# harukaki/brl

Hardware: AMD Instinct MI355X
Metric: env-steps/sec at num_envs=8192, 32-step rollout, 1/2/4/8 MI355X (higher is better)
Workload: dtype u8

## Files before the change

brl_amd/_capi.py:

```python
from __future__ import annotations

import ctypes as C
import os

_PKG = os.path.dirname(os.path.abspath(__file__))
LIB_PATH = os.path.join(_PKG, "lib", "libbrl_hip.so")

STATE_WORDS = 16
OBS_SIZE = 480
NUM_ACTIONS = 38

_vp = C.c_void_p


class Fields(C.Structure):
    _names = ["current_player", "terminated", "rewards", "step_count", "turn", "dealer", "vul_ns", "vul_ew",
              "shuffled_players", "last_bid", "last_bidder", "call_x", "call_xx", "pass_num",
              "first_denomination_ns", "first_denomination_ew", "hand", "tricks", "lut_idx", "board_ctr", "illegal"]
    _fields_ = [(n, _vp) for n in _names]


class TransitionPtrs(C.Structure):
    _names = ["done", "action", "value", "reward", "log_prob", "obs", "legal_action_mask"]
    _fields_ = [(n, _vp) for n in _names]
# ... 95 lines not shown
        "brl_ppo_stats": [i32, _vp, i64, _vp, f32, f32, _vp, _vp],
        "brl_ppo_heads_loss_split": [i32, _vp, i64, _vp, _vp, i64, _vp, _vp, _vp, _vp, _vp, _vp, i64, f32, f32, f32, i32, i32, i32, _vp, _vp, _vp, _vp, _vp, i32, _vp],
        "brl_ppo_heads_bwd": [i32, _vp, _vp, i64, _vp, i64, i64, i32, i32, _vp, _vp, _vp, _vp, _vp, _vp, i64, _vp, _vp, _vp, _vp],
        "brl_ppo_stats_rows": [i32, _vp, _vp, i64, i64, f32, f32, f32, _vp, _vp],
        "brl_mb_gather_bind": [i32, C.POINTER(TransitionPtrs), _vp, _vp, _vp, _vp, i64, _vp, _vp, _vp, _vp, _vp, _vp, _vp, i64, _vp, _vp],
        "brl_adam_clip_fin_gather": [i32, _vp, _vp, _vp, _vp, i64, _vp, f32, _vp, f32, f32, f32, f32, _vp, i64, _vp, _vp, _vp, i64,
                                     i32, _vp, _vp, _vp, _vp, _vp],
        "brl_mb_gather_dev": [i32, _vp, i64, _vp],
        "brl_ppo_stats_gram": [i32, _vp, i64, i64, _vp, i64, f32, f32, f32, _vp, _vp, _vp, _vp],
        "brl_ppo_illegal_grad": [i32, _vp, _vp, _vp, f32, i64, _vp, _vp],
        "brl_act_bwd_colsum": [i32, _vp, _vp, i64, i64, i64, i32, _vp, _vp],
        "brl_act_bwd_colsum_heads_dw": [i32, _vp, _vp, i64, i64, i64, i32, _vp, _vp, _vp, i64, i64, i64, i32, _vp, _vp, _vp, _vp, i64,
                                        _vp, _vp, _vp, _vp],
        "brl_bias_finalize_ex": [i32, i32, _vp, _vp, _vp, _vp, _vp],
        "brl_bias_finalize_rows": [i32, i32, _vp, _vp, _vp, _vp, i32, _vp, _vp],
        "brl_fair_forward": [i32, C.POINTER(FairNet), _vp, i64, i32, _vp, _vp, _vp],
        "brl_mlp_gemm_group": [i32, i32, i32, _vp, _vp, _vp, _vp, _vp, _vp, _vp, _vp, _vp, _vp],
        "brl_fair_chain": [i32, C.POINTER(FairNet), _vp, _vp, _vp, _vp, _vp, _vp, _vp, i64, f32, f32, f32, i32, i32, i32, i32,
                           C.POINTER(FairWork), _vp],
        "brl_mlp_gemm": [i32, i32, i32, _vp, i64, _vp, i64, _vp, i64, i64, i64, i64, i32, _vp, _vp, i64, _vp, _vp, _vp],
        "brl_mlp_gemm_x3_workspace": [i64, i64, i64, _vp],
        "brl_mlp_gemm_x3_group": [i32, i32, i32, _vp, _vp, _vp, _vp, _vp, _vp, _vp, _vp, _vp, _vp],
        "brl_split_planes": [i32, _vp, i64, _vp, i64, _vp],
        "brl_linear_x3p": [i32, _vp, i32, i64, i64, _vp, i64, i64, _vp, i32, _vp, i64, _vp, i64, i64, i64, i64, i64, _vp],
        "brl_mlp_gemm_x3": [i32, i32, i32, _vp, i64, _vp, i64, _vp, i64, i64, i64, i64, i32, _vp, _vp, i64, _vp, _vp, i64, _vp],
        "brl_mlp_forward_rows": [i32, C.POINTER(MlpRef), _vp, _vp, i64, _vp, i64, _vp, i64, _vp],
        "brl_adam_shard_norm": [i32, _vp, C.POINTER(ShardGeom), i32, i32, f32, _vp, _vp, _vp, _vp],
        "brl_adam_shard_apply": [i32, _vp, _vp, _vp, _vp, C.POINTER(ShardGeom), i32, i32, _vp, _vp, f32, _vp, f32, f32, f32, f32, f32, _vp,
                                 _vp, i64, _vp],
        "brl_mlp_gemm_dh_heads_dw": [i32, _vp, i64, _vp, i64, _vp, i64, i64, i64, i64, i32, _vp, i64, _vp, _vp, _vp, i64, i64, i64, i32,
                                     _vp, _vp, _vp, _vp, i64, _vp, _vp, _vp, _vp],
    }
    sigs.update(sl_signatures())
    for name, args in sigs.items():
        fn = getattr(L, name)
        fn.argtypes = args
        fn.restype = i32
    _lib = L
    return L


EXPORTS = ["brl_last_error", "brl_version", "brl_create", "brl_set_lut", "brl_destroy", "brl_set_rng",
           "brl_init_random", "brl_init_from_deals", "brl_step", "brl_observe", "brl_get_fields",
           "brl_rollout_random", "brl_policy_step", "brl_policy_step_at", "brl_obs_cast", "brl_obs_cast_rows", "brl_live_index", "brl_linear_act", "brl_linear_act_heads", "brl_gae", "brl_imp_reward", "brl_duplicate_step",
           "brl_eval_step", "brl_eval_reduce", "brl_ppo_loss", "brl_ppo_stats", "brl_policy_step_ex",
           "brl_eval_step_team", "brl_rollout_random_gae", "brl_ppo_heads_loss_split", "brl_adam_shard_norm", "brl_adam_shard_apply", "brl_ppo_heads_bwd", "brl_ppo_stats_gram",
           "brl_act_bwd_colsum", "brl_act_bwd_colsum_heads_dw", "brl_bias_finalize_ex", "brl_ppo_stats_rows", "brl_mb_gather_bind", "brl_mb_gather_dev", "brl_ppo_illegal_grad", "brl_adam_clip_fin_gather", "brl_mlp_gemm", "brl_mlp_gemm_dh_heads_dw", "brl_mlp_forward_rows",
           "brl_bias_finalize_rows", "brl_fair_chain", "brl_mlp_gemm_group", "brl_fair_forward", "brl_mlp_gemm_x3", "brl_mlp_gemm_x3_workspace", "brl_mlp_gemm_x3_group", "brl_split_planes", "brl_linear_x3p"]


def sl_signatures() -> dict:
    i64, i32, u64, f32 = C.c_int64, C.c_int, C.c_uint64, C.c_float
    return {
        "brl_sl_sample": [i32, _vp, _vp, i64, u64, i64, _vp, _vp, _vp],
        "brl_sl_replay": [i32, _vp, _vp, _vp, i64, _vp, _vp, i64, _vp, _vp, _vp, _vp],
        "brl_sl_loss": [i32, _vp, i64, _vp, _vp, i64, f32, _vp, _vp, _vp, i64, _vp],
    }


def check(rc: int) -> None:
    if rc != 0:
        raise BrlError(f"libbrl_hip error {rc}: {lib().brl_last_error().decode()}")


def ptr(t):
    if t is None:
        return None
    assert t.is_contiguous(), "brl_amd passes raw pointers: tensors must be contiguous"
    return t.data_ptr()
```

brl_amd/csrc/brl_mlp_gemm_x3.hip:

```cpp
#include <hip/hip_runtime.h>
#include <stdint.h>

#include "abi_common.hpp"
#include "mlp_gemm_x3.hpp"
#include "mlp_linear_x3p.hpp"

static int64_t x3_tiles(int64_t m, int64_t n) { return ((m + 127) / 128) * ((n + 127) / 128); }

static int64_t x3_workspace_bytes(int64_t m, int64_t n, int64_t k) {
  const int sk = mgs::pick_splitk(m, n, k);
  if (sk == 1) return 0;
  const int64_t tiles = x3_tiles(m, n);
  return ((tiles * 4 + 255) / 256) * 256 + tiles * sk * (int64_t)mgs::SLAB_FLOATS * 4;
}

extern "C" int brl_mlp_gemm_x3_workspace(int64_t m, int64_t n, int64_t k, int64_t *bytes) {
  NEED(bytes && m > 0 && n > 0 && k > 0, "bytes / m / n / k");
  *bytes = x3_workspace_bytes(m, n, k);
  return BRL_OK;
}

extern "C" int brl_mlp_gemm_x3(int device, int layout, int epilogue, const float *a, int64_t lda, const float *b, int64_t ldb, float *c,
                               int64_t ldc, int64_t m, int64_t n, int64_t k, int act, const float *bias, const float *gate, int64_t ldg,
                               float *colsum, void *workspace, int64_t workspace_bytes, void *stream) {
  NEED(a && b && c && m > 0 && n > 0 && k > 0, "a / b / c / m / n / k");
  NEED(layout >= BRL_GEMM_NT && layout <= BRL_GEMM_TN, "layout (BRL_GEMM_NT / _NN / _TN)");
  NEED(m < (1 << 24) && n < (1 << 24) && k < (1 << 24), "m / n / k below 2^24");
  NEED(n % 4 == 0 && ldc % 4 == 0 && lda % 4 == 0 && ldb % 4 == 0 && ldc >= n, "n and the leading dimensions multiples of 4 (16-byte pieces)");
  const bool akc = layout != BRL_GEMM_TN, bkc = layout == BRL_GEMM_NT;
  NEED(k % 32 == 0, "k a multiple of 32 (whole 32-deep chunks; other k: brl_mlp_gemm)");
  NEED(akc ? lda >= k : lda >= ((m + 3) & ~(int64_t)3), "lda (where m is contiguous in a: at least m rounded up to 4 — whole 16-byte pieces are read)");
  NEED(bkc ? ldb >= k : ldb >= n, "ldb");
  NEED((akc ? m * lda : k * lda) < (1ll << 29) && (bkc ? n * ldb : k * ldb) < (1ll << 29), "operands below 2 GB");
  NEED(act == 0 || act == 1, "act (0 ReLU, 1 tanh)");
  NEED((epilogue == BRL_GEMM_EPI_NONE) || (epilogue == BRL_GEMM_EPI_BIAS_ACT && layout == BRL_GEMM_NT && bias) ||
           (epilogue == BRL_GEMM_EPI_GATE_COLSUM && layout == BRL_GEMM_NN && gate && ldg >= n && ldg % 4 == 0),
// ... 44 lines not shown
    NEED(m[i] < (1 << 24) && n[i] < (1 << 24) && k[i] < (1 << 24), "m / n / k below 2^24");
    NEED(n[i] % 4 == 0 && ldc[i] % 4 == 0 && lda[i] % 4 == 0 && ldb[i] % 4 == 0 && ldc[i] >= n[i], "n and the leading dimensions multiples of 4");
    NEED(k[i] % 32 == 0, "k a multiple of 32 (whole 32-deep chunks; other k: brl_mlp_gemm_group)");
    NEED(akc ? lda[i] >= k[i] : lda[i] >= ((m[i] + 3) & ~(int64_t)3), "lda (where m is contiguous in a: at least m rounded up to 4)");
    NEED(bkc ? ldb[i] >= k[i] : ldb[i] >= n[i], "ldb");
    NEED((akc ? m[i] * lda[i] : k[i] * lda[i]) < (1ll << 29) && (bkc ? n[i] * ldb[i] : k[i] * ldb[i]) < (1ll << 29), "operands below 2 GB");
    NEED((((uintptr_t)a[i] | (uintptr_t)b[i] | (uintptr_t)c[i]) & 15) == 0, "16-byte alignment");
    mgs::Args &X = GA.x[i];
    mg::Args &G = X.g;
    G.A = a[i]; G.lda = lda[i]; G.B = b[i]; G.ldb = ldb[i]; G.C = c[i]; G.ldc = ldc[i];
    G.M = (int)m[i]; G.N = (int)n[i]; G.K = (int)k[i];
    X.splitk = 1;
    GA.first[i + 1] = GA.first[i] + (int)x3_tiles(m[i], n[i]);
  }
  HIP_TRY(hipSetDevice(device));
  hipStream_t s = (hipStream_t)stream;
  const unsigned blocks = (unsigned)GA.first[count];
  if (layout == BRL_GEMM_NT) hipLaunchKernelGGL((mgs::k_gemm_x3s_group<true, true>), dim3(blocks), dim3(mgs::THREADS), 0, s, GA);
  else if (layout == BRL_GEMM_NN) hipLaunchKernelGGL((mgs::k_gemm_x3s_group<true, false>), dim3(blocks), dim3(mgs::THREADS), 0, s, GA);
  else hipLaunchKernelGGL((mgs::k_gemm_x3s_group<false, false>), dim3(blocks), dim3(mgs::THREADS), 0, s, GA);
  HIP_TRY(hipGetLastError());
  return BRL_OK;
}

extern "C" int brl_split_planes(int device, const float *x, int64_t n, uint16_t *planes, int64_t plane_stride, void *stream) {
  NEED(x && planes && n > 0 && n % 4 == 0 && plane_stride >= n && plane_stride % 4 == 0, "x / planes / n (a multiple of 4) / plane_stride");
  NEED((((uintptr_t)x) & 15) == 0 && (((uintptr_t)planes) & 7) == 0, "alignment (x 16 bytes, planes 8)");
  HIP_TRY(hipSetDevice(device));
  hipLaunchKernelGGL(lx3::k_split_planes, dim3((unsigned)((n / 4 + 255) / 256)), dim3(256), 0, (hipStream_t)stream, x, planes, plane_stride, n / 4);
  HIP_TRY(hipGetLastError());
  return BRL_OK;
}

extern "C" int brl_linear_x3p(int device, const uint16_t *x_planes, int npx, int64_t ldx, int64_t sx, const uint16_t *w_planes, int64_t ldw,
                              int64_t sw, const float *bias, int relu, float *y, int64_t ldy, uint16_t *y_planes, int64_t ldyp, int64_t syp,
                              int64_t m, int64_t n, int64_t k, void *stream) {
  NEED(x_planes && w_planes && bias && (y || y_planes) && m > 0 && n > 0 && k > 0, "x_planes / w_planes / bias / an output / m / n / k");
  NEED(npx == 1 || npx == 3, "npx (3 planes, or 1: x exact in bf16)");
  NEED(n % 128 == 0 && k % 32 == 0, "n a multiple of 128, k a multiple of 32");
  NEED(m < (1 << 24) && n < (1 << 24) && k < (1 << 24), "m / n / k below 2^24");
  NEED(ldx >= k && ldx % 8 == 0 && ldw >= k && ldw % 8 == 0, "ldx / ldw (at least k, multiples of 8: 16-byte pieces)");
  NEED(m * ldx < (1ll << 31) && n * ldw < (1ll << 31), "planes below 4 GB each");
  NEED(!y || (ldy >= n && ldy % 4 == 0), "ldy");
  NEED(!y_planes || (ldyp >= n && ldyp % 8 == 0 && syp % 8 == 0), "ldyp / syp (multiples of 8)");
  NEED(sx % 8 == 0 && sw % 8 == 0, "plane strides multiples of 8");
  NEED((((uintptr_t)x_planes | (uintptr_t)w_planes | (uintptr_t)bias | (uintptr_t)y | (uintptr_t)y_planes) & 15) == 0, "16-byte alignment");
  HIP_TRY(hipSetDevice(device));
  lx3::Args G{};
  G.x = x_planes; G.ldx = ldx; G.sx = sx; G.w = w_planes; G.ldw = ldw; G.sw = sw; G.bias = bias;
  G.y = y; G.ldy = ldy; G.yp = y_planes; G.ldyp = ldyp; G.syp = syp;
  G.M = (int)m; G.N = (int)n; G.K = (int)k; G.relu = relu ? 1 : 0;
  hipStream_t s = (hipStream_t)stream;
  const unsigned blocks = (unsigned)(((m + 127) / 128) * (n / 128));
  if (npx == 3) hipLaunchKernelGGL(lx3::k_linear_x3p<3>, dim3(blocks), dim3(lx3::THREADS), 0, s, G);
  else hipLaunchKernelGGL(lx3::k_linear_x3p<1>, dim3(blocks), dim3(lx3::THREADS), 0, s, G);
  HIP_TRY(hipGetLastError());
  return BRL_OK;
}
```

brl_amd/csrc/mlp_linear_x3p.hpp:

```cpp
#pragma once

#include "mlp_gemm.hpp"

namespace lx3 {

using mg::f32x4;
typedef __bf16 bf16x8 __attribute__((ext_vector_type(8)));
typedef float f32x16 __attribute__((ext_vector_type(16)));
typedef unsigned u32x4 __attribute__((ext_vector_type(4)));
typedef unsigned u32x2 __attribute__((ext_vector_type(2)));

constexpr int BK = 32, STAGES = 3, THREADS = 512;
constexpr int PLANE = 128 * 64;
constexpr int STAGE_BYTES = 6 * PLANE;
constexpr int LDS_BYTES = STAGES * STAGE_BYTES;
constexpr int C_ROW_BYTES = 128 * 2 + 16;
static_assert(3 * 128 * C_ROW_BYTES <= LDS_BYTES, "the output planes reuse the stages");

struct Args {
  const uint16_t *x;
  int64_t ldx, sx;
  const uint16_t *w;
  int64_t ldw, sw;
  const float *bias;
  float *y;
  int64_t ldy;
  uint16_t *yp;
  int64_t ldyp, syp;
  int M, N, K;
  int relu;
#ifdef LX3_TIMING
  unsigned long long *dbg;
#endif
};
#ifdef LX3_TIMING
#define LX3_STAMP(k) do { if (threadIdx.x == 0 && G.dbg) { G.dbg[(size_t)blockIdx.x * 4 + 2 * (k)] = __builtin_amdgcn_s_memtime(); \
                                                          G.dbg[(size_t)blockIdx.x * 4 + 2 * (k) + 1] = __builtin_amdgcn_s_memrealtime(); } } while (0)
#else
#define LX3_STAMP(k) do { } while (0)
#endif

template <bool V>
struct BoolTag { static constexpr bool value = V; };

#ifndef LX3_STORE
#define LX3_STORE 0
#endif
#ifndef LX3_EXP
#define LX3_EXP 0
#endif

__device__ __forceinline__ void glds16(const void *g, void *lds_wave_base) {
  __builtin_amdgcn_global_load_lds((const __attribute__((address_space(1))) void *)g, (__attribute__((address_space(3))) void *)lds_wave_base, 16,
                                   0, 0);
}

__device__ __forceinline__ void split3(const float x, unsigned &hi, unsigned &mid, unsigned &lo) {
  const unsigned u = __float_as_uint(x);
  const float r = x - __uint_as_float(u & 0xffff0000u);
  const unsigned ur = __float_as_uint(r);
  const float l = r - __uint_as_float(ur & 0xffff0000u);
  hi = u >> 16;
  mid = ur >> 16;
  lo = __float_as_uint(l) >> 16;
}

template <int NPX>
__global__ __launch_bounds__(THREADS) void k_linear_x3p(Args G) {
  static_assert(NPX == 1 || NPX == 3, "x: one plane (exact in bf16) or three");
  constexpr int NI = NPX + 3;
  constexpr int NP = NPX == 3 ? 6 : 3;
  constexpr int NMF = 4 * NP;
  constexpr int NFR = 2 * NPX + 3;
  __shared__ __attribute__((aligned(16))) unsigned char lds[LDS_BYTES];
  const int tid = (int)threadIdx.x, lane = tid & 63, w = __builtin_amdgcn_readfirstlane(tid >> 6);
  const int tiles_m = (G.M + 127) / 128, tiles_n = G.N / 128, nblk = (int)gridDim.x, bid = (int)blockIdx.x;
  const int L = (nblk % 8 == 0) ? (bid % 8) * (nblk / 8) + bid / 8 : bid;
  int tm, tn;
  if (tiles_m % 2 == 0 && tiles_n % 4 == 0) {
    const int blk = L >> 3, i = L & 7;
    tm = 2 * (blk / (tiles_n / 4)) + (i >> 2);
    tn = 4 * (blk % (tiles_n / 4)) + (i & 3);
  } else {
    tm = L / tiles_n;
    tn = L - tm * tiles_n;
  }
  const int m0 = tm * 128, n0 = tn * 128;
  const int nchunks = G.K / BK;

  uint32_t offx, offw;
  {
    const int row = 16 * w + (lane >> 2), pc = (lane & 3) ^ ((row >> 2) & 3);
    const int mr = (m0 + row < G.M) ? m0 + row : G.M - 1;
    offx = (uint32_t)(((int64_t)mr * G.ldx + 8 * pc) * 2);
    offw = (uint32_t)(((int64_t)(n0 + row) * G.ldw + 8 * pc) * 2);
  }
  int kc = 0;
  auto stage_one = [&](unsigned char *st, int j) __attribute__((always_inline)) {
    const bool isw = j >= NPX;
    const char *base = reinterpret_cast<const char *>(isw ? G.w + (int64_t)(j - NPX) * G.sw : G.x + (int64_t)j * G.sx);
// ... 93 lines not shown
    for (int t = 1; t < NMF; t++) {
      mf(fu, t);
      __builtin_amdgcn_sched_barrier(0);
      if (t - 1 < NI && dma) stage_one(st, t - 1);
      if (t - 1 < 2 * NFR && next && !(LX3_EXP & 4)) {
        int s, u;
        rorder(t - 1, s, u);
        fn[s][u] = read_frag(sn, s, u);
      }
      __builtin_amdgcn_sched_barrier(0);
    }
    if (dma) kc++;
  };
  static_assert(2 * NFR <= NMF - 1, "a fragment read per gap");
  {
    using T = BoolTag<true>;
    using F = BoolTag<false>;
    const int nfull = nchunks - 3;
    int c = 0, stage = 0;
    auto nxt = [&]() { stage = (stage + 1 == STAGES) ? 0 : stage + 1; };
    for (; c + 1 < nfull; c += 2) {
      phase(T{}, f0, f1, c, stage); nxt();
      phase(T{}, f1, f0, c + 1, stage); nxt();
    }
    for (; c + 1 < nchunks; c += 2) {
      phase(F{}, f0, f1, c, stage); nxt();
      phase(F{}, f1, f0, c + 1, stage); nxt();
    }
    if (c < nchunks) phase(F{}, f0, f1, c, stage);
  }

  LX3_STAMP(1);
  __syncthreads();
  const float floor_v = G.relu ? 0.0f : -__builtin_inff();
#pragma unroll
  for (int b = 0; b < 2; b++) {
    const int row = 64 * wm + 32 * b + r32, em = m0 + row;
#pragma unroll
    for (int g = 0; g < 4; g++) {
      const int col = 32 * wn + 8 * g + 4 * hh;
      const f32x4 bias4 = *reinterpret_cast<const f32x4 *>(G.bias + n0 + col);
      f32x4 o;
#pragma unroll
      for (int e = 0; e < 4; e++) o[e] = fmaxf((acc[b][1][4 * g + e] + acc[b][0][4 * g + e]) + bias4[e], floor_v);
      if (G.y != nullptr && em < G.M) *reinterpret_cast<f32x4 *>(G.y + (int64_t)em * G.ldy + n0 + col) = o;
      if (G.yp != nullptr) {
        unsigned h[4], m[4], l[4];
#pragma unroll
        for (int e = 0; e < 4; e++) split3(o[e], h[e], m[e], l[e]);
        unsigned char *p = lds + row * C_ROW_BYTES + col * 2;
        *reinterpret_cast<u32x2 *>(p) = u32x2{h[0] | (h[1] << 16), h[2] | (h[3] << 16)};
        *reinterpret_cast<u32x2 *>(p + 128 * C_ROW_BYTES) = u32x2{m[0] | (m[1] << 16), m[2] | (m[3] << 16)};
        *reinterpret_cast<u32x2 *>(p + 2 * 128 * C_ROW_BYTES) = u32x2{l[0] | (l[1] << 16), l[2] | (l[3] << 16)};
      }
    }
  }
  if (G.yp != nullptr) {
    __syncthreads();
#pragma unroll
    for (int it = 0; it < (3 * 128 * 16) / THREADS; it++) {
      const int idx = it * THREADS + tid, pl = idx >> 11, row = (idx >> 4) & 127, ch = idx & 15;
      const u32x4 v = *reinterpret_cast<const u32x4 *>(lds + (pl * 128 + row) * C_ROW_BYTES + ch * 16);
      if (m0 + row < G.M) {
        u32x4 *dst = reinterpret_cast<u32x4 *>(G.yp + (int64_t)pl * G.syp + (int64_t)(m0 + row) * G.ldyp + n0 + ch * 8);
#if LX3_STORE == 1
        __builtin_nontemporal_store(v, dst);
#elif LX3_STORE == 2
        asm volatile("global_store_dwordx4 %0, %1, off sc0 sc1" ::"v"(dst), "v"(v) : "memory");
#else
        *dst = v;
#endif
      }
    }
  }
}

__global__ __launch_bounds__(256) void k_split_planes(const float *x, uint16_t *planes, int64_t stride, int64_t n4) {
  const int64_t idx = (int64_t)blockIdx.x * 256 + threadIdx.x;
  if (idx >= n4) return;
  const f32x4 v = reinterpret_cast<const f32x4 *>(x)[idx];
  unsigned h[4], m[4], l[4];
#pragma unroll
  for (int e = 0; e < 4; e++) split3(v[e], h[e], m[e], l[e]);
  uint16_t *p = planes + 4 * idx;
  *reinterpret_cast<u32x2 *>(p) = u32x2{h[0] | (h[1] << 16), h[2] | (h[3] << 16)};
  *reinterpret_cast<u32x2 *>(p + stride) = u32x2{m[0] | (m[1] << 16), m[2] | (m[3] << 16)};
  *reinterpret_cast<u32x2 *>(p + 2 * stride) = u32x2{l[0] | (l[1] << 16), l[2] | (l[3] << 16)};
}

}
// ... 1 lines not shown
```

brl_amd/models.py:

```python
from __future__ import annotations

import math
import os

import torch
import torch.nn as nn


def _haiku_linear(fan_in: int, fan_out: int) -> nn.Linear:
    lin = nn.Linear(fan_in, fan_out)
    std = 1.0 / math.sqrt(fan_in)
    nn.init.trunc_normal_(lin.weight, mean=0.0, std=std, a=-2 * std, b=2 * std)
    nn.init.zeros_(lin.bias)
    return lin


class ActorCritic(nn.Module):
    def __init__(self, action_dim: int = 38, activation: str = "relu", model: str = "DeepMind", obs_dim: int = 480):
        super().__init__()
        self.model = model
        self.act = torch.relu if activation == "relu" else torch.tanh
        if model.startswith("DeepMind"):
            depth = int(model.split("_")[1]) if "_" in model else 4
            self.body = nn.ModuleList([_haiku_linear(obs_dim, 1024)] + [_haiku_linear(1024, 1024) for _ in range(depth - 1)])
# ... 80 lines not shown
class InferenceSnapshot:

    def __init__(self, module: "ActorCritic", dtype=None, env=None, own_cast=True, views=False, gemm=None):
        self.env = env
        self.own_cast = bool(own_cast)
        self.dtype = dtype or torch.float32
        dt = self.dtype
        self.gemm_x3 = (gemm or os.environ.get("BRL_INFERENCE_GEMM", "") or "bf16x3") == "bf16x3" and dt == torch.float32 \
            and all(lin.weight.shape[1] % 32 == 0 and lin.weight.shape[0] % 4 == 0 for lin in module.body)
        self.lin = None
        self.wp = None
        if self.gemm_x3:
            self.lin = [(lin.weight.detach(), lin.bias.detach()) if views else (lin.weight.detach().clone(), lin.bias.detach().clone())
                        for lin in module.body]
            if os.environ.get("BRL_INFERENCE_PLANES", "1") != "0" and all(
                    w.is_cuda and w.dtype == torch.float32 and w.is_contiguous() and w.shape[0] % 128 == 0 and w.shape[1] % 32 == 0
                    and w.data_ptr() % 16 == 0 and b.data_ptr() % 16 == 0 for w, b in self.lin):
                self.wp = [torch.empty((3,) + tuple(w.shape), dtype=torch.bfloat16, device=w.device) for w, _ in self.lin]
                self._split_weights()
        self.views = bool(views) and dt == torch.float32 and all(lin.weight.dtype == torch.float32 for lin in module.body)
        if self.views:
            self.body = [(lin.weight.detach().t(), lin.bias.detach()) for lin in module.body]
        else:
            self.body = [(lin.weight.detach().to(dt).t().contiguous(), lin.bias.detach().to(dt)) for lin in module.body]
        self.n_actions = module.actor.weight.shape[0]
        self.head_b = torch.cat([module.actor.bias, module.critic.bias], 0).detach().to(dt)
        if self.views:
            self.head_wt = torch.cat([module.actor.weight, module.critic.weight], 0).detach()
            self.head_w = self.head_wt.t()
        else:
            self.head_w = torch.cat([module.actor.weight, module.critic.weight], 0).detach().to(dt).t().contiguous()
            self.head_wt = self.head_w.t().contiguous()
        self.head_bf = self.head_b.float().contiguous()
        self.body_nk = None
        if env is not None and dt in (torch.bfloat16, torch.float16) and os.environ.get("BRL_LINEAR16", "1") != "0" \
                and all(lin.weight.shape[0] % 128 == 0 and lin.weight.shape[1] % 8 == 0 for lin in module.body):
            self.body_nk = [(lin.weight.detach().to(dt).contiguous(), lin.bias.detach().to(dt).float().contiguous())
                            for lin in module.body]

    def refresh(self, module: "ActorCritic"):
        if self.body_nk is not None:
            return self._refresh16(module)
        if self.lin is not None:
            if self.views:
                self.lin = [(lin.weight.detach(), lin.bias.detach()) for lin in module.body]
            else:
                for (w, b), lin in zip(self.lin, module.body):
                    w.copy_(lin.weight.detach())
                    b.copy_(lin.bias.detach())
            if self.wp is not None:
                self._split_weights()
        if self.views:
            self.body = [(lin.weight.detach().t(), lin.bias.detach()) for lin in module.body]
        else:
            for (w, b), lin in zip(self.body, module.body):
                w.copy_(lin.weight.detach().t())
                b.copy_(lin.bias.detach())
        k = self.n_actions
        self.head_w[:, :k].copy_(module.actor.weight.detach().t())
        self.head_w[:, k:].copy_(module.critic.weight.detach().t())
        self.head_b[:k].copy_(module.actor.bias.detach())
        self.head_b[k:].copy_(module.critic.bias.detach())
        if not self.views:
            self.head_wt.copy_(self.head_w.t())
        self.head_bf.copy_(self.head_b)

    def _split_weights(self):
        from . import _capi
        L = _capi.lib()
        for (w, _), wp in zip(self.lin, self.wp):
            di = w.device.index if w.device.index is not None else torch.cuda.current_device()
            _capi.check(L.brl_split_planes(di, w.data_ptr(), w.numel(), wp.data_ptr(), w.numel(),
                                           torch.cuda.current_stream(w.device).cuda_stream))

    def planes_for(self, n):
        return self.wp is not None and n >= 4096

    def _body_planes(self, x):
        from . import _capi
        L, st = _capi.lib(), torch.cuda.current_stream(x.device).cuda_stream
        di = x.device.index if x.device.index is not None else torch.cuda.current_device()
        n, k = x.shape
        xp, npx, sx = x, 1, 0
        y = None
        for li, ((w, b), wp) in enumerate(zip(self.lin, self.wp)):
            out, last = w.shape[0], li + 1 == len(self.lin)
            y = torch.empty((n, out), dtype=torch.float32, device=x.device) if last else None
            yp = None if last else torch.empty((3, n, out), dtype=torch.bfloat16, device=x.device)
            _capi.check(L.brl_linear_x3p(di, xp.data_ptr(), npx, k, sx, wp.data_ptr(), k, out * k, b.data_ptr(), 1,
                                         y.data_ptr() if last else None, out, None if last else yp.data_ptr(), out, n * out, n, out, k, st))
            xp, npx, sx, k = yp, 3, n * out, out
        return y

    def _refresh16(self, module):
        k = self.n_actions

        def copy_all(dst, src):
            if hasattr(torch, "_foreach_copy_"):
                torch._foreach_copy_(dst, src)
            else:
                for d, s_ in zip(dst, src):
                    d.copy_(s_)

        with torch.no_grad():
            ws = [w for w, _ in self.body_nk] + [self.head_wt[:k], self.head_wt[k:]]
            src = [lin.weight.detach() for lin in module.body] + [module.actor.weight.detach(), module.critic.weight.detach()]
            copy_all(ws, src)
            b16 = [b for _, b in self.body] + [self.head_b[:k], self.head_b[k:]]
            copy_all(b16, [lin.bias.detach() for lin in module.body] + [module.actor.bias.detach(), module.critic.bias.detach()])
            copy_all([b for _, b in self.body_nk] + [self.head_bf], [b for _, b in self.body] + [self.head_b])
            self.head_w.copy_(self.head_wt.t())
        self._body_stale = True

    @staticmethod
    def covers(module):
        return str(getattr(module, "model", "")).startswith("DeepMind") and getattr(module, "act", None) is torch.relu

    @staticmethod
    def make(module, dtype=None, env=None, own_cast=True, views=False, gemm=None):
# ... 27 lines not shown
            for w, b in self.body_nk:
                y = torch.empty((x.shape[0], w.shape[0]), dtype=self.dtype, device=x.device)
                _capi.check(L.brl_linear_act(self.env._h, x.data_ptr(), x.stride(0), w.data_ptr(), w.stride(0), b.data_ptr(),
                                           y.data_ptr(), y.stride(0), x.shape[0], w.shape[0], w.shape[1], 1, fmt, st))
                x = y
            return x
        if x.dim() == 2 and self.planes_for(x.shape[0]) and x.is_cuda and x.is_contiguous() and x.data_ptr() % 16 == 0 \
                and x.dtype == torch.bfloat16 and self.dtype == torch.float32:
            return self._body_planes(x)
        if x.dtype != self.dtype:
            raise RuntimeError(f"InferenceSnapshot: input in {x.dtype} where the layers run in {self.dtype} (bf16 input is taken by the "
                               "planes path only: >= 4096 contiguous rows)")
        if self.gemm_x3 and x.is_cuda and x.dim() == 2 and x.shape[0] >= 4096 and x.is_contiguous() and x.data_ptr() % 16 == 0:
            from . import _capi
            L, st = _capi.lib(), torch.cuda.current_stream(x.device).cuda_stream
            di = x.device.index if x.device.index is not None else torch.cuda.current_device()
            for w, b in self.lin:
                y = torch.empty((x.shape[0], w.shape[0]), dtype=torch.float32, device=x.device)
                _capi.check(L.brl_mlp_gemm_x3(di, 0, 1, x.data_ptr(), x.stride(0), w.data_ptr(), w.stride(0), y.data_ptr(), y.stride(0),
                                              x.shape[0], w.shape[0], w.shape[1], 0, b.data_ptr(), None, 0, None, None, 0, st))
                x = y
            return x
        if getattr(self, "_body_stale", False):
            for (w, _), (wn, _) in zip(self.body, self.body_nk):
                w.copy_(wn.t())
            self._body_stale = False
        fused = hasattr(torch, "_addmm_activation")
        for w, b in self.body:
            x = torch._addmm_activation(b, x, w, use_gelu=False) if fused else torch.addmm(b, x, w).relu_()
        return x

    HEAD_PART_LD = 40

    def head_parts(self, obs, x=None):
        if self.body_nk is None or os.environ.get("BRL_HEAD_PARTS", "1") == "0":
            return None
        if x is None:
            x = self._input(obs)
        if not (x.is_cuda and x.dim() == 2 and x.is_contiguous() and x.shape[0] > 0):
            return None
        from . import _capi
        from .bridge_bidding import _stream
        L, fmt, st, n = _capi.lib(), self._FMT[self.dtype], _stream(), x.shape[0]
        for w, b in self.body_nk[:-1]:
            y = torch.empty((n, w.shape[0]), dtype=self.dtype, device=x.device)
            _capi.check(L.brl_linear_act(self.env._h, x.data_ptr(), x.stride(0), w.data_ptr(), w.stride(0), b.data_ptr(),
                                         y.data_ptr(), y.stride(0), n, w.shape[0], w.shape[1], 1, fmt, st))
            x = y
        w, b = self.body_nk[-1]
        parts = torch.empty((w.shape[0] // 128, n, self.HEAD_PART_LD), dtype=torch.float32, device=x.device)
        _capi.check(L.brl_linear_act_heads(self.env._h, x.data_ptr(), x.stride(0), w.data_ptr(), w.stride(0), b.data_ptr(), None, 0,
                                           n, w.shape[0], w.shape[1], 1, fmt, self.head_wt.data_ptr(), self.head_wt.stride(0),
                                           self.head_wt.shape[0], parts.data_ptr(), parts.stride(1), parts.stride(0), st))
        return parts

    def hidden(self, obs, x=None):
        if x is None:
            x = self._input(obs)
        return self._body(x)

    def heads(self, obs, x=None, raw=False):
        if x is None:
            x = self._input(obs)
        x = self._body(x)
        out = torch.addmm(self.head_b, x, self.head_w)
        return out if raw else out.float()

    def __call__(self, obs):
        out = self.heads(obs)
# ... 24 lines not shown
```

brl_amd/roll_out.py:

```python
from __future__ import annotations

import ctypes as C
from typing import NamedTuple

import torch

from . import _capi
from ._capi import NUM_ACTIONS, OBS_SIZE, check, ptr
from .bridge_bidding import BridgeBidding, State, _stream
from .models import InferenceSnapshot
from .utils import MODE, SAMPLE, UNMASKED, _pass_logits, policy_step


class Transition(NamedTuple):
    done: torch.Tensor
    action: torch.Tensor
    value: torch.Tensor
    reward: torch.Tensor
    log_prob: torch.Tensor
    obs: torch.Tensor
    legal_action_mask: torch.Tensor


def alloc_transition(T: int, n: int, device) -> Transition:
# ... 97 lines not shown
        self.sub_actions = e((T, 3, n), torch.int32)
        self.draw = torch.zeros(1, dtype=torch.int32, device=dev)
        self.tc = torch.zeros(1, dtype=torch.int64, device=dev)
        self.xin = e((n, OBS_SIZE), self.infer_dtype or torch.float32)
        self.scale = torch.tensor(self.reward_scale, dtype=torch.float32, device=dev)

    def _bind(self, params, opp_params):
        if self.static:
            if self.snap_actor is None:
                self.snap_actor = InferenceSnapshot.make(params, self.infer_dtype, self.env, gemm=self.gemm)
                self.snap_opp = InferenceSnapshot.make(opp_params, self.infer_dtype, self.env, gemm=self.gemm)
            else:
                self.snap_actor.refresh(params)
                self.snap_opp.refresh(opp_params)
        else:
            self.snap_actor = InferenceSnapshot.make(params, self.infer_dtype, self.env, own_cast=False, gemm=self.gemm)
            self.snap_opp = self.snap_actor if opp_params is params \
                else InferenceSnapshot.make(opp_params, self.infer_dtype, self.env, own_cast=False, gemm=self.gemm)
        self.params, self.opp_params = params, opp_params
        consumers = [self.snap_actor] + ([self.snap_opp] if self.game_mode == "competitive" else [])
        want = self.infer_dtype or torch.float32
        if self.infer_dtype is None and all(sn is not None and sn.planes_for(self.n) for sn in consumers):
            want = torch.bfloat16
        if getattr(self, "xin", None) is not None and self.xin.dtype != want:
            if self.graphs is not None:
                raise RuntimeError("the captured rollout holds the observation buffer in " + str(self.xin.dtype))
            self.xin = torch.empty((self.n, OBS_SIZE), dtype=want, device=self.env.device)

    _FMT = {torch.float32: 0, torch.bfloat16: 1, torch.float16: 2}

    def _fused_heads(self, is_opp):
        import os
        snap = self.snap_opp if is_opp else self.snap_actor
        ok = snap is not None and self.fuse_heads and self.infer_dtype in (torch.bfloat16, torch.float16) \
            and os.environ.get("BRL_TABLES_PER_WAVE", "4") == "4"
        return snap if ok else None

    def _heads_input(self, snap, obs, x):
        parts = snap.head_parts(obs, x)
        return parts if parts is not None else snap.hidden(obs, x)

    def _head_ext(self, snap, h, **kw):
        if h.dim() == 3:
            return _capi.MacroExt(head_part=h.data_ptr(), head_part_stride=h.stride(0), head_part_ld=h.stride(1),
                                  head_nparts=h.shape[0], head_b=snap.head_bf.data_ptr(), **kw)
        return _capi.MacroExt(head_h=h.data_ptr(), head_ldh=h.stride(0), head_w=snap.head_wt.data_ptr(), head_b=snap.head_bf.data_ptr(),
                              head_hidden=h.shape[1], head_fmt=self._FMT[h.dtype], **kw)

    def _forward(self, is_opp, obs_bool, x=None):
        snap = self.snap_opp if is_opp else self.snap_actor
        if snap is not None:
            out = snap.heads(obs_bool, x, raw=True)
            return out[:, :snap.n_actions], out[:, snap.n_actions]
        fp, pr = (self.opp_fp, self.opp_params) if is_opp else (self.actor_fp, self.params)
        if self.infer_dtype is None:
            return fp.apply(pr, obs_bool.to(torch.float32) if x is None else x)
        with torch.autocast("cuda", dtype=self.infer_dtype):
            lg, v = fp.apply(pr, obs_bool.to(self.infer_dtype) if x is None else x)
        return lg.float(), v.float()

    def _macro_step(self, t):
        env, traj, packed, cur = self.env, self.traj, self.packed, self.cur
        racc, tacc, T = self.racc, self.tacc, self.T
        competitive = self.game_mode == "competitive"
        MX = _capi.MacroExt
        fmt = self._FMT[self.xin.dtype]
        actor = cur[t & 1]
        mode1 = SAMPLE if self.masked else SAMPLE | UNMASKED
        snap = self._fused_heads(False)
        if snap is not None:
            h = self._heads_input(snap, traj.obs[t], None if t == 0 else self.xin)
            policy_step(env, packed, packed, None, mode1, 4 * t, True, action=traj.action[t], log_prob=traj.log_prob[t],
# ... 134 lines not shown
```

Baseline: 10.73 billion.

## Fuse policy/value head partial products into the last split-plane body linear

Adds a HEADS variant of the three-plane bf16 linear kernel. The last body layer's output tile stays in LDS and is immediately multiplied by the split head weights with MFMA, writing per-tile partial head products instead of the full fp32 hidden activations. The fp32 rollout path now routes through this fused-heads path when observations are bf16 and planes apply. This removes a write and reread of the hidden layer and a separate head GEMM, in exchange for extra LDS, register use and a new hard error if the fused path does not apply.

```diff
diff --git a/brl_amd/_capi.py b/brl_amd/_capi.py
--- a/brl_amd/_capi.py
+++ b/brl_amd/_capi.py
@@ -151,6 +151,7 @@
                                      _vp, _vp, _vp, _vp, i64, _vp, _vp, _vp, _vp],
     }
     sigs.update(sl_signatures())
+    sigs.update(x3p_signatures())
     for name, args in sigs.items():
         fn = getattr(L, name)
         fn.argtypes = args
@@ -177,6 +178,13 @@
     }
 
 
+def x3p_signatures() -> dict:
+    i64, i32 = C.c_int64, C.c_int
+    return {
+        "brl_linear_x3p_heads": [i32, _vp, i32, i64, i64, _vp, i64, i64, _vp, i32, _vp, i64, i64, i32, _vp, i64, i64, i64, i64, i64, _vp],
+    }
+
+
 def check(rc: int) -> None:
     if rc != 0:
         raise BrlError(f"libbrl_hip error {rc}: {lib().brl_last_error().decode()}")
diff --git a/brl_amd/csrc/brl_mlp_gemm_x3.hip b/brl_amd/csrc/brl_mlp_gemm_x3.hip
--- a/brl_amd/csrc/brl_mlp_gemm_x3.hip
+++ b/brl_amd/csrc/brl_mlp_gemm_x3.hip
@@ -2,6 +2,7 @@
 #include <stdint.h>
 
 #include "abi_common.hpp"
+#include "../../include/brl_x3p.h"
 #include "mlp_gemm_x3.hpp"
 #include "mlp_linear_x3p.hpp"
 
@@ -112,28 +113,61 @@
   return BRL_OK;
 }
 
-extern "C" int brl_linear_x3p(int device, const uint16_t *x_planes, int npx, int64_t ldx, int64_t sx, const uint16_t *w_planes, int64_t ldw,
-                              int64_t sw, const float *bias, int relu, float *y, int64_t ldy, uint16_t *y_planes, int64_t ldyp, int64_t syp,
-                              int64_t m, int64_t n, int64_t k, void *stream) {
-  NEED(x_planes && w_planes && bias && (y || y_planes) && m > 0 && n > 0 && k > 0, "x_planes / w_planes / bias / an output / m / n / k");
+static int x3p_args(lx3::Args &G, const uint16_t *x_planes, int npx, int64_t ldx, int64_t sx, const uint16_t *w_planes, int64_t ldw,
+                    int64_t sw, const float *bias, int relu, int64_t m, int64_t n, int64_t k) {
+  NEED(x_planes && w_planes && bias && m > 0 && n > 0 && k > 0, "x_planes / w_planes / bias / m / n / k");
   NEED(npx == 1 || npx == 3, "npx (3 planes, or 1: x exact in bf16)");
   NEED(n % 128 == 0 && k % 32 == 0, "n a multiple of 128, k a multiple of 32");
   NEED(m < (1 << 24) && n < (1 << 24) && k < (1 << 24), "m / n / k below 2^24");
   NEED(ldx >= k && ldx % 8 == 0 && ldw >= k && ldw % 8 == 0, "ldx / ldw (at least k, multiples of 8: 16-byte pieces)");
   NEED(m * ldx < (1ll << 31) && n * ldw < (1ll << 31), "planes below 4 GB each");
-  NEED(!y || (ldy >= n && ldy % 4 == 0), "ldy");
-  NEED(!y_planes || (ldyp >= n && ldyp % 8 == 0 && syp % 8 == 0), "ldyp / syp (multiples of 8)");
   NEED(sx % 8 == 0 && sw % 8 == 0, "plane strides multiples of 8");
-  NEED((((uintptr_t)x_planes | (uintptr_t)w_planes | (uintptr_t)bias | (uintptr_t)y | (uintptr_t)y_planes) & 15) == 0, "16-byte alignment");
-  HIP_TRY(hipSetDevice(device));
-  lx3::Args G{};
+  NEED((((uintptr_t)x_planes | (uintptr_t)w_planes | (uintptr_t)bias) & 15) == 0, "16-byte alignment");
+  G = lx3::Args{};
   G.x = x_planes; G.ldx = ldx; G.sx = sx; G.w = w_planes; G.ldw = ldw; G.sw = sw; G.bias = bias;
-  G.y = y; G.ldy = ldy; G.yp = y_planes; G.ldyp = ldyp; G.syp = syp;
   G.M = (int)m; G.N = (int)n; G.K = (int)k; G.relu = relu ? 1 : 0;
-  hipStream_t s = (hipStream_t)stream;
-  const unsigned blocks = (unsigned)(((m + 127) / 128) * (n / 128));
-  if (npx == 3) hipLaunchKernelGGL(lx3::k_linear_x3p<3>, dim3(blocks), dim3(lx3::THREADS), 0, s, G);
-  else hipLaunchKernelGGL(lx3::k_linear_x3p<1>, dim3(blocks), dim3(lx3::THREADS), 0, s, G);
+  return BRL_OK;
+}
+
+template <bool HEADS>
+static int x3p_launch(const lx3::Args &G, int npx, hipStream_t s) {
+  const unsigned blocks = (unsigned)(((G.M + 127) / 128) * (G.N / 128));
+  if (npx == 3) hipLaunchKernelGGL((lx3::k_linear_x3p<3, HEADS>), dim3(blocks), dim3(lx3::THREADS), 0, s, G);
+  else hipLaunchKernelGGL((lx3::k_linear_x3p<1, HEADS>), dim3(blocks), dim3(lx3::THREADS), 0, s, G);
   HIP_TRY(hipGetLastError());
   return BRL_OK;
 }
+
+extern "C" int brl_linear_x3p(int device, const uint16_t *x_planes, int npx, int64_t ldx, int64_t sx, const uint16_t *w_planes, int64_t ldw,
+                              int64_t sw, const float *bias, int relu, float *y, int64_t ldy, uint16_t *y_planes, int64_t ldyp, int64_t syp,
+                              int64_t m, int64_t n, int64_t k, void *stream) {
+  NEED(y || y_planes, "an output");
+  lx3::Args G;
+  if (int rc = x3p_args(G, x_planes, npx, ldx, sx, w_planes, ldw, sw, bias, relu, m, n, k)) return rc;
+  NEED(!y || (ldy >= n && ldy % 4 == 0), "ldy");
+  NEED(!y_planes || (ldyp >= n && ldyp % 8 == 0 && syp % 8 == 0), "ldyp / syp (multiples of 8)");
+  NEED((((uintptr_t)y | (uintptr_t)y_planes) & 15) == 0, "16-byte alignment");
+  HIP_TRY(hipSetDevice(device));
+  G.y = y; G.ldy = ldy; G.yp = y_planes; G.ldyp = ldyp; G.syp = syp;
+  return x3p_launch<false>(G, npx, (hipStream_t)stream);
+}
+
+extern "C" int brl_linear_x3p_heads(int device, const uint16_t *x_planes, int npx, int64_t ldx, int64_t sx, const uint16_t *w_planes,
+                                    int64_t ldw, int64_t sw, const float *bias, int relu, const uint16_t *head_w_planes, int64_t ld_head_w,
+                                    int64_t head_w_stride, int n_heads, float *head_part, int64_t head_part_ld, int64_t head_part_stride,
+                                    int64_t m, int64_t n, int64_t k, void *stream) {
+  lx3::Args G;
+  if (int rc = x3p_args(G, x_planes, npx, ldx, sx, w_planes, ldw, sw, bias, relu, m, n, k)) return rc;
+  NEED(head_w_planes && head_part, "head_w_planes / head_part");
+  NEED(n_heads >= 1 && n_heads <= lx3::HW_ROWS, "n_heads (1..48)");
+  NEED(ld_head_w >= n && ld_head_w % 8 == 0 && head_w_stride >= n_heads * ld_head_w && head_w_stride % 8 == 0,
+       "ld_head_w (at least n, a multiple of 8) / head_w_stride (at least n_heads * ld_head_w, a multiple of 8)");
+  NEED(head_part_ld >= ((n_heads + 3) & ~3) && head_part_ld % 4 == 0 && head_part_stride >= m * head_part_ld && head_part_stride % 4 == 0,
+       "head_part_ld (a multiple of 4, at least n_heads rounded up to 4) / head_part_stride (at least m * head_part_ld, a multiple of 4)");
+  NEED(3 * head_w_stride < (1ll << 31) && (n / 128) * head_part_stride < (1ll << 31), "head weight planes / partial products below 2^31 elements");
+  NEED((((uintptr_t)head_w_planes | (uintptr_t)head_part) & 15) == 0, "16-byte alignment");
+  HIP_TRY(hipSetDevice(device));
+  G.hw = head_w_planes; G.ld_hw = ld_head_w; G.shw = head_w_stride; G.n_heads = n_heads;
+  G.head_part = head_part; G.head_part_ld = head_part_ld; G.head_part_stride = head_part_stride;
+  return x3p_launch<true>(G, npx, (hipStream_t)stream);
+}
diff --git a/brl_amd/csrc/mlp_linear_x3p.hpp b/brl_amd/csrc/mlp_linear_x3p.hpp
--- a/brl_amd/csrc/mlp_linear_x3p.hpp
+++ b/brl_amd/csrc/mlp_linear_x3p.hpp
@@ -16,6 +16,10 @@
 constexpr int LDS_BYTES = STAGES * STAGE_BYTES;
 constexpr int C_ROW_BYTES = 128 * 2 + 16;
 static_assert(3 * 128 * C_ROW_BYTES <= LDS_BYTES, "the output planes reuse the stages");
+constexpr int HW_ROWS = 48;
+constexpr int HW_OFF = 3 * 128 * C_ROW_BYTES;
+constexpr int HW_PIECES = 3 * HW_ROWS * 16;
+static_assert(HW_OFF + 3 * HW_ROWS * C_ROW_BYTES <= LDS_BYTES, "y's planes and the heads' weight planes share the stages");
 
 struct Args {
   const uint16_t *x;
@@ -29,6 +33,11 @@
   int64_t ldyp, syp;
   int M, N, K;
   int relu;
+  const uint16_t *hw;
+  int64_t ld_hw, shw;
+  int n_heads;
+  float *head_part;
+  int64_t head_part_ld, head_part_stride;
 #ifdef LX3_TIMING
   unsigned long long *dbg;
 #endif
@@ -65,7 +74,7 @@
   lo = __float_as_uint(l) >> 16;
 }
 
-template <int NPX>
+template <int NPX, bool HEADS>
 __global__ __launch_bounds__(THREADS) void k_linear_x3p(Args G) {
   static_assert(NPX == 1 || NPX == 3, "x: one plane (exact in bf16) or three");
   constexpr int NI = NPX + 3;
@@ -225,6 +234,18 @@
 
   LX3_STAMP(1);
   __syncthreads();
+  constexpr int HW_IT = HEADS ? (HW_PIECES + THREADS - 1) / THREADS : 1;
+  u32x4 hwv[HW_IT];
+  if (HEADS) {
+#pragma unroll
+    for (int it = 0; it < HW_IT; it++) {
+      const int idx = it * THREADS + tid, pl = idx / (HW_ROWS * 16), hrow = (idx >> 4) % HW_ROWS, ch = idx & 15;
+      hwv[it] = u32x4{0u, 0u, 0u, 0u};
+      if (idx < HW_PIECES && hrow < G.n_heads)
+        hwv[it] = *reinterpret_cast<const u32x4 *>(G.hw + (int64_t)pl * G.shw + (int64_t)hrow * G.ld_hw + n0 + ch * 8);
+    }
+  }
+  const bool planes = HEADS || G.yp != nullptr;
   const float floor_v = G.relu ? 0.0f : -__builtin_inff();
 #pragma unroll
   for (int b = 0; b < 2; b++) {
@@ -236,8 +257,8 @@
       f32x4 o;
 #pragma unroll
       for (int e = 0; e < 4; e++) o[e] = fmaxf((acc[b][1][4 * g + e] + acc[b][0][4 * g + e]) + bias4[e], floor_v);
-      if (G.y != nullptr && em < G.M) *reinterpret_cast<f32x4 *>(G.y + (int64_t)em * G.ldy + n0 + col) = o;
-      if (G.yp != nullptr) {
+      if (!HEADS && G.y != nullptr && em < G.M) *reinterpret_cast<f32x4 *>(G.y + (int64_t)em * G.ldy + n0 + col) = o;
+      if (planes) {
         unsigned h[4], m[4], l[4];
 #pragma unroll
         for (int e = 0; e < 4; e++) split3(o[e], h[e], m[e], l[e]);
@@ -248,7 +269,48 @@
       }
     }
   }
-  if (G.yp != nullptr) {
+  if (HEADS) {
+#pragma unroll
+    for (int it = 0; it < HW_IT; it++) {
+      const int idx = it * THREADS + tid, pl = idx / (HW_ROWS * 16), hrow = (idx >> 4) % HW_ROWS, ch = idx & 15;
+      if (idx < HW_PIECES) *reinterpret_cast<u32x4 *>(lds + HW_OFF + (pl * HW_ROWS + hrow) * C_ROW_BYTES + ch * 16) = hwv[it];
+    }
+    __syncthreads();
+    const int r = lane & 15, kq = lane >> 4;
+    f32x4 hacc[2][3];
+#pragma unroll
+    for (int c = 0; c < 2; c++)
+#pragma unroll
+      for (int nb = 0; nb < 3; nb++) hacc[c][nb] = f32x4{0.f, 0.f, 0.f, 0.f};
+#pragma unroll
+    for (int ks = 0; ks < 4; ks++) {
+      bf16x8 yf[3], hf[3][3];
+#pragma unroll
+      for (int p = 0; p < 3; p++)
+        yf[p] = __builtin_bit_cast(bf16x8, *reinterpret_cast<const u32x4 *>(lds + (p * 128 + 16 * w + r) * C_ROW_BYTES + 64 * ks + 16 * kq));
+#pragma unroll
+      for (int p = 0; p < 3; p++)
+#pragma unroll
+        for (int nb = 0; nb < 3; nb++)
+          hf[p][nb] = __builtin_bit_cast(bf16x8, *reinterpret_cast<const u32x4 *>(lds + HW_OFF + (p * HW_ROWS + 16 * nb + r) * C_ROW_BYTES +
+                                                                                 64 * ks + 16 * kq));
+      constexpr int PW[6] = {2, 0, 1, 1, 0, 0}, PY[6] = {0, 2, 1, 0, 1, 0};
+#pragma unroll
+      for (int q = 0; q < 6; q++)
+#pragma unroll
+        for (int nb = 0; nb < 3; nb++) {
+          const int cls = q == 5 ? 0 : 1;
+          hacc[cls][nb] = __builtin_amdgcn_mfma_f32_16x16x32_bf16(hf[PW[q]][nb], yf[PY[q]], hacc[cls][nb], 0, 0, 0);
+        }
+    }
+    const int m = m0 + 16 * w + r;
+    float *part = G.head_part + (int64_t)tn * G.head_part_stride;
+#pragma unroll
+    for (int nb = 0; nb < 3; nb++) {
+      const int n = 16 * nb + 4 * kq;
+      if (n < G.n_heads && m < G.M) *reinterpret_cast<f32x4 *>(part + (int64_t)m * G.head_part_ld + n) = hacc[1][nb] + hacc[0][nb];
+    }
+  } else if (G.yp != nullptr) {
     __syncthreads();
 #pragma unroll
     for (int it = 0; it < (3 * 128 * 16) / THREADS; it++) {
diff --git a/brl_amd/models.py b/brl_amd/models.py
--- a/brl_amd/models.py
+++ b/brl_amd/models.py
@@ -136,6 +136,11 @@
             self.head_w = torch.cat([module.actor.weight, module.critic.weight], 0).detach().to(dt).t().contiguous()
             self.head_wt = self.head_w.t().contiguous()
         self.head_bf = self.head_b.float().contiguous()
+        self.hwp = None
+        if self.wp is not None and self.head_wt.dtype == torch.float32 and self.head_wt.is_contiguous() and self.head_wt.shape[0] <= 48 \
+                and self.head_wt.shape[1] == self.lin[-1][0].shape[0] and self.head_wt.numel() % 8 == 0 and self.head_wt.data_ptr() % 16 == 0:
+            self.hwp = torch.empty((3,) + tuple(self.head_wt.shape), dtype=torch.bfloat16, device=self.head_wt.device)
+            self._split_heads()
         self.body_nk = None
         if env is not None and dt in (torch.bfloat16, torch.float16) and os.environ.get("BRL_LINEAR16", "1") != "0" \
                 and all(lin.weight.shape[0] % 128 == 0 and lin.weight.shape[1] % 8 == 0 for lin in module.body):
@@ -168,6 +173,8 @@
         if not self.views:
             self.head_wt.copy_(self.head_w.t())
         self.head_bf.copy_(self.head_b)
+        if self.hwp is not None:
+            self._split_heads()
 
     def _split_weights(self):
         from . import _capi
@@ -177,10 +184,17 @@
             _capi.check(L.brl_split_planes(di, w.data_ptr(), w.numel(), wp.data_ptr(), w.numel(),
                                            torch.cuda.current_stream(w.device).cuda_stream))
 
+    def _split_heads(self):
+        from . import _capi
+        w = self.head_wt
+        di = w.device.index if w.device.index is not None else torch.cuda.current_device()
+        _capi.check(_capi.lib().brl_split_planes(di, w.data_ptr(), w.numel(), self.hwp.data_ptr(), w.numel(),
+                                                 torch.cuda.current_stream(w.device).cuda_stream))
+
     def planes_for(self, n):
         return self.wp is not None and n >= 4096
 
-    def _body_planes(self, x):
+    def _body_planes(self, x, heads=False):
         from . import _capi
         L, st = _capi.lib(), torch.cuda.current_stream(x.device).cuda_stream
         di = x.device.index if x.device.index is not None else torch.cuda.current_device()
@@ -189,6 +203,13 @@
         y = None
         for li, ((w, b), wp) in enumerate(zip(self.lin, self.wp)):
             out, last = w.shape[0], li + 1 == len(self.lin)
+            if last and heads:
+                hw = self.hwp
+                parts = torch.empty((out // 128, n, self.HEAD_PART_LD), dtype=torch.float32, device=x.device)
+                _capi.check(L.brl_linear_x3p_heads(di, xp.data_ptr(), npx, k, sx, wp.data_ptr(), k, out * k, b.data_ptr(), 1,
+                                                   hw.data_ptr(), hw.shape[2], hw.stride(0), hw.shape[1], parts.data_ptr(), parts.stride(1),
+                                                   parts.stride(0), n, out, k, st))
+                return parts
             y = torch.empty((n, out), dtype=torch.float32, device=x.device) if last else None
             yp = None if last else torch.empty((3, n, out), dtype=torch.bfloat16, device=x.device)
             _capi.check(L.brl_linear_x3p(di, xp.data_ptr(), npx, k, sx, wp.data_ptr(), k, out * k, b.data_ptr(), 1,
@@ -282,9 +303,21 @@
 
     HEAD_PART_LD = 40
 
+    def parts_for(self, n):
+        return self.hwp is not None and self.planes_for(n) and os.environ.get("BRL_HEAD_PARTS", "1") != "0"
+
     def head_parts(self, obs, x=None):
-        if self.body_nk is None or os.environ.get("BRL_HEAD_PARTS", "1") == "0":
-            return None
+        if os.environ.get("BRL_HEAD_PARTS", "1") == "0":
+            return None
+        if self.body_nk is None:
+            if self.hwp is None:
+                return None
+            if x is None:
+                x = self._input(obs)
+            if not (x.dim() == 2 and self.parts_for(x.shape[0]) and x.is_cuda and x.is_contiguous() and x.data_ptr() % 16 == 0
+                    and x.dtype == torch.bfloat16):
+                return None
+            return self._body_planes(x, heads=True)
         if x is None:
             x = self._input(obs)
         if not (x.is_cuda and x.dim() == 2 and x.is_contiguous() and x.shape[0] > 0):
diff --git a/brl_amd/roll_out.py b/brl_amd/roll_out.py
--- a/brl_amd/roll_out.py
+++ b/brl_amd/roll_out.py
@@ -153,12 +153,15 @@
     def _fused_heads(self, is_opp):
         import os
         snap = self.snap_opp if is_opp else self.snap_actor
-        ok = snap is not None and self.fuse_heads and self.infer_dtype in (torch.bfloat16, torch.float16) \
-            and os.environ.get("BRL_TABLES_PER_WAVE", "4") == "4"
+        ok = snap is not None and self.fuse_heads and os.environ.get("BRL_TABLES_PER_WAVE", "4") == "4" and (
+            self.infer_dtype in (torch.bfloat16, torch.float16)
+            or (self.infer_dtype is None and self.xin.dtype == torch.bfloat16 and snap.parts_for(self.n)))
         return snap if ok else None
 
     def _heads_input(self, snap, obs, x):
         parts = snap.head_parts(obs, x)
+        if parts is None and self.infer_dtype is None:
+            raise RuntimeError("fp32 rollout: the heads' partial products (brl_linear_x3p_heads) did not apply")
         return parts if parts is not None else snap.hidden(obs, x)
 
     def _head_ext(self, snap, h, **kw):
diff --git a/include/brl_x3p.h b/include/brl_x3p.h
--- /dev/null
+++ b/include/brl_x3p.h
@@ -0,0 +1,19 @@
+#ifndef BRL_X3P_H
+#define BRL_X3P_H
+
+#include <stdint.h>
+
+#ifdef __cplusplus
+extern "C" {
+#endif
+
+int brl_linear_x3p_heads(int device, const uint16_t *x_planes, int npx, int64_t ldx, int64_t sx, const uint16_t *w_planes, int64_t ldw,
+                         int64_t sw, const float *bias, int relu, const uint16_t *head_w_planes, int64_t ld_head_w, int64_t head_w_stride,
+                         int n_heads, float *head_part, int64_t head_part_ld, int64_t head_part_stride, int64_t m, int64_t n, int64_t k,
+                         void *stream);
+
+#ifdef __cplusplus
+}
+#endif
+
+#endif
```

Result: no change. 10.73 billion, median of 4 (-0.0%).
